# emilieparent/pypulsar

Hardware: AMD Instinct MI355X
Metric: DM-trial samples*channels/sec (node) + % HBM roofline (higher is better)
Workload: dtype u8

## Files before the change

### include/pdd.h

```cpp
#ifndef PDD_H
#define PDD_H

#include <stdint.h>

#ifdef __cplusplus
extern "C" {
#endif

enum { PDD_F32 = 0, PDD_U8 = 1, PDD_U16 = 2 };
enum {
  PDD_PAD_VALUE = 0,
  PDD_PAD_ROTATE = 1
};
enum { PDD_STAT_MEAN = 0, PDD_STAT_MEDIAN = 1, PDD_STAT_STD = 2, PDD_STAT_MIN = 3, PDD_STAT_MAX = 4 };
enum { PDD_LAYOUT_TIME_MAJOR = 0,
       PDD_LAYOUT_CHAN_MAJOR = 1   };

int pdd_version(void);
const char* pdd_last_error(void);
const char* pdd_source_digest(void);
int pdd_scratch_release(void);
int pdd_sync(void* stream);

int pdd_corner_turn(const void* in, int in_dtype, int64_t nspec, int64_t nchan, int64_t ld_in,
// ... 48 lines not shown
#define PDD_SWEEP_FACTOR_FORCE 2
#define PDD_SWEEP_FACTOR_G2 4
#define PDD_SWEEP_FACTOR_G4 8
#define PDD_SWEEP_NO_SKEW 16
int pdd_sweep_plan_create_ex(const int32_t* host_table, int64_t D, int64_t C, int dtype, int flags,
                             pdd_sweep_plan** plan);
int pdd_sweep_plan_factor(const pdd_sweep_plan* plan, int64_t* n_patterns);
int pdd_sweep_plan_skew(const pdd_sweep_plan* plan, int64_t* extra_tiles);
int pdd_sweep_execute(const pdd_sweep_plan* plan, const void* x, int64_t N, int64_t ld,
                      int pad_mode, const float* padvals, float* out, int64_t ld_out,
                      int64_t n_out, void* stream);
int pdd_sweep_execute_ex(const pdd_sweep_plan* plan, const void* x, int64_t N, int64_t ld,
                         int64_t piece, int64_t x_off, int pad_mode, const float* padvals,
                         float* out, int64_t ld_out, int64_t n_out, float out_bias,
                         void* stream);
int64_t pdd_sweep_pattern_bytes(const pdd_sweep_plan* plan, int64_t n_out);
int pdd_sweep_execute_stage(const pdd_sweep_plan* plan, const void* x, int64_t N, int64_t ld,
                            int64_t piece, int64_t x_off, int pad_mode, const float* padvals,
                            float* out, int64_t ld_out, int64_t n_out, float out_bias,
                            void* patterns, int64_t pattern_bytes, int stage, void* stream);
int pdd_stream_create_cu_mask(const uint32_t* mask, int n_words, void** stream);
int pdd_stream_destroy(void* stream);
int pdd_sweep_plan_create_grouped(const int32_t* host_table, int64_t n_grp, int64_t D, int64_t C,
                                  int dtype, pdd_sweep_plan** plan);
int pdd_sweep_execute_grouped(const pdd_sweep_plan* plan, const void* x, int64_t N, int64_t ld,
                              int pad_mode, const float* padvals, float* out, int64_t ld_out,
                              int64_t n_out, int64_t row_g, int64_t row_d, void* stream);
int pdd_sweep_execute_ds(const pdd_sweep_plan* plan, const uint8_t* x8, int64_t n_raw, int64_t ld,
                         int64_t ds, int pad_mode, const float* padvals, float* out,
                         int64_t ld_out, int64_t n_out, int64_t row_g, int64_t row_d,
// ... 80 lines not shown
```

### pypulsar_amd/_lib.py

```python
import ctypes
import os

import torch

from . import _digest

_HERE = os.path.dirname(os.path.abspath(__file__))
LIB_PATH = os.path.join(_HERE, "libpdd.so")
_DEV_LIB = os.environ.get("PDD_DEV_LIB")
if _DEV_LIB:
    LIB_PATH = _DEV_LIB

F32, U8, U16 = 0, 1, 2
PAD_VALUE, PAD_ROTATE = 0, 1
STAT_MEAN, STAT_MEDIAN, STAT_STD, STAT_MIN, STAT_MAX = 0, 1, 2, 3, 4
LAYOUT_TIME_MAJOR, LAYOUT_CHAN_MAJOR = 0, 1
ENOCHAIN = -5
ZDM_NONE, ZDM_INT, ZDM_WRAP = 0, 1, 2
SWEEP_FACTOR = 1
SWEEP_FACTOR_FORCE = 2
SWEEP_FACTOR_G2 = 4
SWEEP_FACTOR_G4 = 8
SWEEP_NO_SKEW = 16

# ... 3 lines not shown
    "pdd_zero_dm", "pdd_sweep_plan_create", "pdd_sweep_execute", "pdd_sweep_plan_info",
    "pdd_sweep_plan_set_input_max",
    "pdd_sweep_plan_destroy", "pdd_global_stats", "pdd_scale_rows", "pdd_masked_fill",
    "pdd_smooth", "pdd_zdm_downsample", "pdd_sweep_set_timing", "pdd_sweep_kernel_ms",
    "pdd_sweep_plan_create_grouped", "pdd_sweep_execute_grouped", "pdd_sp_chunk_stats",
    "pdd_sp_search", "pdd_psrfits_subints", "pdd_downsample_u8", "pdd_sweep_timing_read",
    "pdd_sweep_execute_ex", "pdd_zdm_int_downsample", "pdd_downsample_u8_u16",
    "pdd_sweep_execute_ds", "pdd_subband_chain", "pdd_scratch_release",
    "pdd_sweep_plan_create_ex", "pdd_sweep_plan_factor", "pdd_sweep_plan_skew", "pdd_source_digest",
    "pdd_sweep_plan_set_poison", "pdd_sweep_plan_set_segment_bytes",
    "pdd_sweep_pattern_bytes", "pdd_sweep_execute_stage", "pdd_stream_create_cu_mask",
    "pdd_stream_destroy", "pdd_ps_prep", "pdd_ps_block_medians", "pdd_ps_normalise",
    "pdd_ps_harmsum", "pdd_ps_search", "pdd_fold_rows", "pdd_fold_search",
    "pdd_acc_correlate", "pdd_acc_search", "pdd_rfi_stats_prep", "pdd_rfi_stats_power",
    "pdd_rfi_apply", "pdd_ffa_plan_info", "pdd_ffa_downsample", "pdd_ffa_detrend", "pdd_ffa_pass",
    "pdd_ffa_search",
)


def source_digest():
    return _digest.source_digest()


class PddLibraryMissing(RuntimeError):
    pass


class PddError(RuntimeError):
    pass


# ... 12 lines not shown
    "pdd_convert_f32": ([_vp, _int, _i64, _i64, _i64, _vp, _i64, _vp], _int),
    "pdd_channel_stats": ([_vp, _i64, _i64, _i64, _int, _vp, _vp], _int),
    "pdd_shift_pad": ([_vp, _i64, _i64, _i64, _vp, _int, _vp, _vp, _i64, _i64, _vp], _int),
    "pdd_shift_group_sum": ([_vp, _i64, _i64, _i64, _vp, _int, _vp, _i64, _vp, _i64, _i64, _vp],
                            _int),
    "pdd_downsample": ([_vp, _i64, _i64, _i64, _i64, _vp, _i64, _vp], _int),
    "pdd_downsample_u8": ([_vp, _i64, _i64, _i64, _i64, _vp, _i64, _vp], _int),
    "pdd_downsample_u8_u16": ([_vp, _i64, _i64, _i64, _i64, _vp, _i64, _vp], _int),
    "pdd_zero_dm": ([_vp, _int, _i64, _i64, _i64, _int, _vp, _i64, _vp], _int),
    "pdd_sweep_plan_create": ([_vp, _i64, _i64, _int, ctypes.POINTER(_vp)], _int),
    "pdd_sweep_plan_create_ex": ([_vp, _i64, _i64, _int, _int, ctypes.POINTER(_vp)], _int),
    "pdd_sweep_plan_factor": ([_vp, _vp], _int),
    "pdd_sweep_plan_skew": ([_vp, _vp], _int),
    "pdd_sweep_execute": ([_vp, _vp, _i64, _i64, _int, _vp, _vp, _i64, _i64, _vp], _int),
    "pdd_sweep_execute_ex": ([_vp, _vp, _i64, _i64, _i64, _i64, _int, _vp, _vp, _i64, _i64,
                              ctypes.c_float, _vp], _int),
    "pdd_sweep_plan_info": ([_vp, _vp], _int),
    "pdd_sweep_pattern_bytes": ([_vp, _i64], _i64),
    "pdd_sweep_execute_stage": ([_vp, _vp, _i64, _i64, _i64, _i64, _int, _vp, _vp, _i64, _i64,
                                 ctypes.c_float, _vp, _i64, _int, _vp], _int),
    "pdd_stream_create_cu_mask": ([_vp, _int, ctypes.POINTER(_vp)], _int),
    "pdd_stream_destroy": ([_vp], _int),
    "pdd_sweep_plan_set_input_max": ([_vp, _int], _int),
    "pdd_sweep_plan_destroy": ([_vp], _int),
    "pdd_global_stats": ([_vp, _i64, _i64, _i64, _vp, _vp], _int),
    "pdd_scale_rows": ([_vp, _i64, _i64, _i64, _vp, _i64, _vp, _i64, _vp, _i64, _vp], _int),
    "pdd_masked_fill": ([_vp, _i64, _i64, _i64, _vp, _i64, _vp, _vp, _i64, _vp], _int),
    "pdd_smooth": ([_vp, _i64, _i64, _i64, _i64, _int, _vp, _vp, _i64, _vp], _int),
    "pdd_zdm_downsample": ([_vp, _int, _i64, _i64, _i64, _i64, _int, _vp, _i64, _vp], _int),
    "pdd_zdm_int_downsample": ([_vp, _int, _i64, _i64, _i64, _i64, _int, _int, _vp, _i64, _vp],
# ... 105 lines not shown
```

### pypulsar_amd/csrc/pdd_sweep.hip

```cpp
#include <algorithm>
#include <cstdio>
#include <cstdlib>
#include <cstring>
#include <type_traits>
#include <vector>

#include "pdd_internal.h"
#include "sweep_plan.h"

namespace pdd {

template <bool U8, int S>
struct ElemOf {
  static constexpr int bytes = U8 ? 2 * S : 4 * S;
  static_assert(bytes == 8 || bytes == 16, "LDS element must be 8 or 16 bytes");
  using type = typename std::conditional<bytes == 8, uint2, uint4>::type;
};

__device__ __forceinline__ uint32_t get_w(const uint2& v, int i) { return i == 0 ? v.x : v.y; }
__device__ __forceinline__ uint32_t get_w(const uint4& v, int i) {
  return i == 0 ? v.x : (i == 1 ? v.y : (i == 2 ? v.z : v.w));
}
__device__ __forceinline__ void set_w(uint2& v, int i, uint32_t x) {
  if (i == 0) v.x = x; else v.y = x;
// ... 354 lines not shown
        "global_load_lds_dwordx4 %1, off\n\t"
        "s_mov_b32 m0, %0"
        : "=&s"(keep)
        : "v"(p), "s"(la)
        : "memory");
  }
}


constexpr int kIlPer = 4;
struct InLayout {
  int64_t ld;
  int64_t piece;
  int psh;
  int64_t pstride;
  __device__ __forceinline__ int64_t at(int c, int64_t s) const {
    return piece ? (s >> psh) * pstride + (int64_t)c * piece + (s & (piece - 1))
                 : (int64_t)c * ld + s;
  }
};

template <typename InT>
struct SrcRows {
  const InT* x;
  InLayout lay;
  __device__ __forceinline__ SrcRows(const void* xv, const InLayout& l)
      : x(static_cast<const InT*>(xv)), lay(l) {}
  __device__ __forceinline__ InT at(int c, int64_t s) const { return x[lay.at(c, s)]; }
};
template <int F, bool VEC>
struct SrcCoadd {
// ... 173 lines not shown

struct FxBatch {
  int y, z, w, lo, hi;
};
__device__ __forceinline__ FxBatch fx_batch(const int4* __restrict__ pat, const int* __restrict__ rng,
                                            int pb, int p1) {
  const int pl = min(pb + (int)(threadIdx.x & 63), p1 - 1);
  const int4 q = pat[pl];
  return {q.y, q.z, q.w, rng[2 * pl], rng[2 * pl + 1]};
}

struct FxS1Args : IlArgs {
  const int4* pat;
  const int* gtab;
  int NG;
};

struct FxFromImage {
  using El = ElemU16;
  static constexpr int kBlock = kFxE;
  static constexpr bool kNontemporal = false;
  const uint4* R;
  int64_t nR;
  __device__ __forceinline__ explicit FxFromImage(const FxS1Args& a)
      : R(static_cast<const uint4*>(a.x)), nR(a.nR) {}
  __device__ __forceinline__ void load_row(uint4* L, int c, int64_t i0, int W) const {
    for (int e = threadIdx.x; e < W; e += 256) {
      const int64_t i = i0 + e;
      L[e] = (i >= 0 && i < nR) ? R[(int64_t)c * nR + i] : make_uint4(0u, 0u, 0u, 0u);
    }
  }
};
template <typename InT>
struct FxFromInput {
  static constexpr bool kF32 = std::is_same<InT, float>::value;
  using El = typename std::conditional<kF32, ElemF32, ElemU16>::type;
  using V = typename El::value_t;
  static constexpr int kBlock = kF32 ? kFxEf : kFxE;
  static constexpr bool kNontemporal = !kF32;
  const SrcRows<InT> src;
  const FxS1Args& a;
  __device__ __forceinline__ explicit FxFromInput(const FxS1Args& a_) : src(a_.x, a_.lay), a(a_) {}
  __device__ __forceinline__ void load_row(typename El::elem_t* L, int c, int64_t i0, int W) const {
    const V pv = pad_value<V>(a.pad_mode, a.padvals, c);
    const int64_t s_lo = a.base + i0, s_hi = s_lo + W - 1 + (El::S - 1) * a.Qs;
// ... 6 lines not shown
        L[e] = El::pack(v);
      }
      return;
    }
    for (int e = threadIdx.x; e < W; e += 256) {
      const int64_t i = i0 + e;
      V v[El::S];
#pragma unroll
      for (int m = 0; m < El::S; ++m) {
        const int64_t sm = a.base + i + m * a.Qs;
        v[m] = (i < 0 || i >= a.nR) ? (V)0 : padded_sample<V>(src, c, sm, a.N, a.pad_mode, pv);
      }
      L[e] = El::pack(v);
    }
  }
};

template <typename Src, int FXG>
__global__ __launch_bounds__(256) void k_fx_stage1(const FxS1Args a) {
  using El = typename Src::El;
  using E = typename El::elem_t;
  constexpr int kE = Src::kBlock;
  extern __shared__ __attribute__((aligned(16))) unsigned char fx_smem[];
  E* L = reinterpret_cast<E*>(fx_smem);
  const int* __restrict__ gtab = a.gtab;
  const int4* __restrict__ pat = a.pat;
  E* __restrict__ P = static_cast<E*>(a.R);
  const int64_t nR = a.nR;
  const int NG = a.NG;
  const int g = blockIdx.x;
  const int64_t j0 = (int64_t)blockIdx.y * kE;
  const int p0 = gtab[g], p1 = gtab[g + 1];
  const int lo = gtab[NG + 1 + 2 * g], hi = gtab[NG + 2 + 2 * g];
  const int W = kE + hi - lo;
  const Src src(a);
  for (int k = 0; k < FXG; ++k) src.load_row(L + k * W, g * FXG + k, j0 + lo, W);
  __syncthreads();
  const int* rng = gtab + 3 * NG + 1;
  for (int pb = p0; pb < p1; pb += 64) {
    const FxBatch B = fx_batch(pat, rng, pb, p1);
    for (int i = 0; i < min(64, p1 - pb); ++i) {
      const int p = pb + i;
      const int4 q = make_int4(0, __builtin_amdgcn_readlane(B.y, i), __builtin_amdgcn_readlane(B.z, i),
                               __builtin_amdgcn_readlane(B.w, i));
      const int64_t jlo = __builtin_amdgcn_readlane(B.lo, i), jhi = nR + __builtin_amdgcn_readlane(B.hi, i);
      if (j0 >= jhi || j0 + kE <= jlo) continue;
#pragma unroll
      for (int e = threadIdx.x; e < kE; e += 256) {
        const int64_t j = j0 + e;
        if (j >= nR) break;
        E s = El::add(L[e - lo], L[W + e - lo + q.y]);
        if constexpr (FXG > 2) {
          s = El::add(s, L[2 * W + e - lo + q.z]);
          s = El::add(s, L[3 * W + e - lo + q.w]);
        }
        E* dst = P + (int64_t)p * nR + j;
        if constexpr (Src::kNontemporal) {
          typedef unsigned int u32x4v __attribute__((ext_vector_type(4)));
          const u32x4v sv = {s.x, s.y, s.z, s.w};
          __builtin_nontemporal_store(sv, reinterpret_cast<u32x4v*>(dst));
        } else {
          *dst = s;
        }
      }
    }
  }
}

typedef void (*fx_s1_fn)(FxS1Args);
constexpr int kFxImage = -1;
struct FxS1Instance {
  int src, fx;
  fx_s1_fn fn;
  int block;
};
#define PDD_FX_S1(SRC_, ...) \
  {SRC_, 2, k_fx_stage1<__VA_ARGS__, 2>, __VA_ARGS__::kBlock}, {SRC_, 4, k_fx_stage1<__VA_ARGS__, 4>, __VA_ARGS__::kBlock}
static const FxS1Instance kFxS1Instances[] = {
    PDD_FX_S1(kFxImage, FxFromImage), PDD_FX_S1(PDD_U8, FxFromInput<uint8_t>),
    PDD_FX_S1(PDD_U16, FxFromInput<uint16_t>), PDD_FX_S1(PDD_F32, FxFromInput<float>)};
#undef PDD_FX_S1

__device__ __forceinline__ int stage_il_dma_win(uint32_t lds_dst, const float4* src, int ne,
                                                int lane) {
  const int nq = (ne + 63) >> 6;
  uint32_t keep;
#define PDD_DMA_RUN(TEXT)                                                                      \
  asm volatile("s_mov_b32 %0, m0\n\ts_mov_b32 m0, %2\n\ts_nop 0\n\t" TEXT "s_mov_b32 m0, %0" \
               : "=&s"(keep) : "v"(s), "s"(m) : "memory")
  for (int q = 0; q < nq; q += 4) {
    const float4* s = src + q * 64 + lane;
    const uint32_t m = __builtin_amdgcn_readfirstlane(lds_dst + q * 1024);
// ... 533 lines not shown

static int debug_flags() { return 0; }

}

struct pdd_sweep_plan : pdd::PlanDims {
  int* d_tab = nullptr;
  int* d_bmin = nullptr;
  int* d_bspan = nullptr;
  int* d_pat = nullptr;
  int* d_wt = nullptr;
  int* d_gtab = nullptr;
  int* d_sig = nullptr;
  int input_max = 0;
  int poison = 0;
  int64_t seg_bytes = 0;
  static constexpr int kEvPairs = 1024;
  hipEvent_t* ev = nullptr;
  int timing = 0;
  int timed = 0;
  int dropped = 0;
};

using namespace pdd;

static void il_lohi(const pdd_sweep_plan* p, int64_t& lo, int64_t& hi) {
  if (p->fx) {
    lo = p->fx_lo;
    hi = (int64_t)p->fx_hi + p->fx_tpad;
  } else {
// ... 82 lines not shown
    const int J = 16 / ds;
    if ((uintptr_t)r.x % 16 == 0 && r.lay.ld % 16 == 0 && b0 % J == 0 && g.Qs % J == 0) vec = 16;
    else if ((uintptr_t)r.x % ds == 0 && r.lay.ld % ds == 0) vec = 1;
  }
  for (const IlInstance& k : kIlInstances) {
    if (k.ds != ds || k.vec != vec || k.dtype != p->dtype || k.u16 != (p->v.S == 8)) continue;
    const IlArgs a{r.x, r.lay, r.N, b0, g.Qs, g.nR, r.pad_mode, r.padvals, r.R};
    hipLaunchKernelGGL(k.fn, dim3((unsigned)cdiv(g.nR, k.per_block), (unsigned)C), dim3(256), 0,
                       r.st, a);
    return hipGetLastError() == hipSuccess ? 0 : il_launch_failed();
  }
  set_error("pdd_sweep_execute: no pre-pass kernel (downsample %d, dtype %d)", ds, p->dtype);
  return -3;
}

static int il_build_patterns(const IlRun& r, const IlSeg& g, int64_t t_base) {
  const pdd_sweep_plan* p = r.p;
  if (p->poison &&
      hipMemsetAsync(r.P, 0xFF, (size_t)(p->n_pat * g.nR) * sizeof(uint4), r.st) != hipSuccess)
    return il_launch_failed();
  if (hipMemsetAsync(r.P + p->n_pat * g.nR, 0, (size_t)g.nR * sizeof(uint4), r.st) != hipSuccess)
    return il_launch_failed();
  if (!p->d_gtab) {
    hipLaunchKernelGGL(k_fx_patterns, dim3((unsigned)p->n_pat, (unsigned)cdiv(g.nR, 256 * kIlPer)),
                       dim3(256), 0, r.st, (const uint4*)r.R, g.nR, (const int4*)p->d_pat, p->fx, r.P);
    return hipGetLastError() == hipSuccess ? 0 : il_launch_failed();
  }
  for (const FxS1Instance& k : kFxS1Instances) {
    if (k.src != (r.fx_direct ? p->dtype : kFxImage) || k.fx != p->fx) continue;
    const int NG = (int)(p->C / p->fx);
    const FxS1Args a{{r.fx_direct ? r.x : r.R, r.lay, r.N, t_base + g.lo + r.x_off, g.Qs, g.nR,
                      r.pad_mode, r.padvals, r.P},
                     (const int4*)p->d_pat, p->d_gtab, NG};
    hipLaunchKernelGGL(k.fn, dim3((unsigned)NG, (unsigned)cdiv(g.nR, k.block)), dim3(256),
                       (size_t)(p->fx * (k.block + p->fx_rspan)) * sizeof(uint4), r.st, a);
    return hipGetLastError() == hipSuccess ? 0 : il_launch_failed();
  }
  set_error("pdd_sweep_execute: no stage-1 kernel (groups of %d, dtype %d)", p->fx, p->dtype);
  return -3;
}

static int il_launch_sweep(const IlRun& r, const IlSeg& g, int64_t t_base, int64_t cnt, float* out,
                           int64_t ld_out, int64_t row_g, int64_t row_d, float out_bias, int flush_n) {
  const pdd_sweep_plan* p = r.p;
  const IlExtra& ex = r.ex;
  const int64_t blocks = g.n_tblk * p->n_dblk * p->n_grp;
  if (blocks >= (1ll << 31)) {
    set_error("pdd_sweep_execute: grid too large");
    return -1;
  }
// ... 91 lines not shown
  if (status != 0) {
    set_error("%s", err.c_str());
    return status;
  }
  pdd_sweep_plan* p = new pdd_sweep_plan();
  static_cast<PlanDims&>(*p) = sp;
  const bool il = p->v.kind == 0;
  hipError_t e = upload(&p->d_tab, il ? sp.meta : sp.rel);
  if (e == hipSuccess) e = upload(&p->d_bmin, il ? sp.chunks : sp.bmin);
  if (e == hipSuccess) e = upload(&p->d_bspan, sp.bspan);
  if (e == hipSuccess && p->fx) e = upload(&p->d_pat, sp.fxt.pat);
  if (e == hipSuccess && p->fx) e = upload(&p->d_wt, sp.fxt.wt);
  if (e == hipSuccess && p->fx_sig_max > 0) e = upload(&p->d_sig, sp.fxt.sig);
  if (e == hipSuccess && !sp.fxt.gtab.empty()) {
    e = upload(&p->d_gtab, sp.fxt.gtab);
    for (const FxS1Instance& k : kFxS1Instances)
      if (e == hipSuccess)
        e = hipFuncSetAttribute((const void*)k.fn, hipFuncAttributeMaxDynamicSharedMemorySize,
                                (int)(4 * (kFxEf + kFxRspan) * sizeof(uint4)));
  }
  if (e != hipSuccess) {
    set_error("pdd_sweep_plan_create: %s", hipGetErrorString(e));
    pdd_sweep_plan_destroy(p);
    return -2;
  }
  if (p->lds_bytes > 64 * 1024) {
    const void* kf = il ? (const void*)il_kernel_for(p->v, p->fx != 0) : (const void*)kernel_for(p->v);
    e = hipFuncSetAttribute(kf, hipFuncAttributeMaxDynamicSharedMemorySize, p->lds_bytes);
    if (e != hipSuccess) {
      set_error("pdd_sweep_plan_create: hipFuncSetAttribute: %s", hipGetErrorString(e));
      pdd_sweep_plan_destroy(p);
      return -2;
    }
  }
// ... 7 lines not shown
  int pad_mode;
  const float* padvals;
};
static int check_execute(const ExecShape& a) {
  PDD_REQUIRE(a.N >= a.N_min && a.n_out >= 0 && a.n_out <= a.n_out_max && a.ld_out >= a.n_out &&
                  a.x_off >= 0 && a.row_g >= 0 && a.row_d >= 0,
              "%s: bad shape", a.fn);
  PDD_REQUIRE(a.piece > 0 || a.ld >= a.ld_min, "%s: row stride %lld < %lld", a.fn, (long long)a.ld,
              (long long)a.ld_min);
  PDD_REQUIRE(a.piece == 0 || (a.piece & (a.piece - 1)) == 0, "%s: piece must be 2^k", a.fn);
  PDD_REQUIRE(a.pad_mode == PDD_PAD_ROTATE || (a.pad_mode == PDD_PAD_VALUE && a.padvals),
              "%s: bad pad mode %d", a.fn, a.pad_mode);
  return 0;
}
static InLayout in_layout(int64_t ld, int64_t piece = 0, int64_t C = 0) {
  InLayout lay{ld, piece, 0, C * piece};
  while ((1ll << lay.psh) < piece) ++lay.psh;
  return lay;
}
constexpr int64_t kAnyColumns = INT64_MAX;

extern "C" {

int pdd_sweep_plan_create(const int32_t* host_table, int64_t D, int64_t C, int dtype,
                          pdd_sweep_plan** plan_out) {
  return plan_create(host_table, 1, D, C, dtype, PDD_SWEEP_FACTOR, plan_out);
}

int pdd_sweep_plan_create_ex(const int32_t* host_table, int64_t D, int64_t C, int dtype, int flags,
                             pdd_sweep_plan** plan_out) {
  return plan_create(host_table, 1, D, C, dtype, flags, plan_out);
// ... 51 lines not shown
              "pdd_sweep_execute: the generic (sparse-grid) kernel reads channel-major input "
              "at offset 0 without an output bias");
  const int64_t n_tblk = cdiv(n_out, p->v.TB());
  const int64_t blocks = n_tblk * p->n_dblk;
  PDD_REQUIRE(blocks < (1ll << 31), "pdd_sweep_execute: grid too large");
  sweep_fn fn = kernel_for(p->v);
  PDD_REQUIRE(fn != nullptr, "pdd_sweep_execute: no kernel");
  hipLaunchKernelGGL(fn, dim3((unsigned)blocks), dim3(p->v.threads()), p->lds_bytes,
                     as_stream(stream), x, ld, (int)p->C, N, p->d_tab, (int)p->Dpad, (int)p->D,
                     p->d_bmin, p->d_bspan, pad_mode, padvals, out, ld_out, n_out, debug_flags(),
                     p->stride, (int)n_tblk, (int)p->n_dblk);
  PDD_LAUNCHED();
  return 0;
}

int64_t pdd_sweep_pattern_bytes(const pdd_sweep_plan* p, int64_t n_out) {
  PDD_REQUIRE(p && n_out >= 0, "pdd_sweep_pattern_bytes: bad arguments");
  if (!p->fx || !p->d_gtab || p->v.kind != 0) return 0;
  return (int64_t)(p->n_pat + 1) * il_seg(p, std::max<int64_t>(n_out, 1)).nR * 16;
}

int pdd_sweep_execute_stage(const pdd_sweep_plan* p, const void* x, int64_t N, int64_t ld,
                            int64_t piece, int64_t x_off, int pad_mode, const float* padvals,
                            float* out, int64_t ld_out, int64_t n_out, float out_bias,
                            void* patterns, int64_t pattern_bytes, int stage, void* stream) {
  PDD_REQUIRE(p && x && patterns && (out || stage == 1), "pdd_sweep_execute_stage: null pointer");
  PDD_REQUIRE(p->fx && p->d_gtab && p->v.kind == 0 && p->n_grp == 1,
              "pdd_sweep_execute_stage: needs a factorised single-group plan");
  PDD_REQUIRE(stage >= 1 && stage <= 3, "pdd_sweep_execute_stage: stage %d not 1, 2 or 3", stage);
  if (int rc = check_execute({"pdd_sweep_execute_stage", N, 1, ld, N, piece, x_off, n_out,
// ... 196 lines not shown
```

### pypulsar_amd/sharding.py

```python
import numpy as np
import torch
import torch.distributed as dist


def dm_slices(D, world, work=None):
    w = np.ones(D) if work is None else np.asarray(work, dtype=np.float64)
    assert len(w) == D and world >= 1
    cum = np.concatenate([[0.0], np.cumsum(w)])
    bounds = [0]
    for r in range(1, world):
        bounds.append(int(np.searchsorted(cum, cum[-1] * r / world, side="left")))
    bounds.append(D)
    bounds = np.maximum.accumulate(bounds)
    return [(int(bounds[r]), int(bounds[r + 1])) for r in range(world)]


def trial_work(dms, downsamp=1):
    d = np.broadcast_to(np.asarray(downsamp, dtype=np.float64), (len(dms),))
    return 1.0 / d


def plan_trial_work(ddplan):
    dms = np.concatenate([np.asarray(s.DMs, dtype=np.float64) for s in ddplan.DDsteps])
    work = np.concatenate([trial_work(s.DMs, s.downsamp) for s in ddplan.DDsteps])
# ... 26 lines not shown
    _all_gather_into(out, part.contiguous(), group=group)
    return out


def _codes():
    from . import _lib
    return {torch.uint8: _lib.U8, torch.float32: _lib.F32}


def _corner_turn(src_tc, dst_cm):
    from ._lib import call, ptr, stream_ptr
    n, C = src_tc.shape
    code = _codes()[src_tc.dtype]
    call("pdd_corner_turn", ptr(src_tc), code, n, C, src_tc.stride(0), ptr(dst_cm), code,
         dst_cm.stride(0), stream_ptr())


class DMShardedSweep(object):

    def __init__(self, dms, freqs, dt, N, dtype=torch.uint8, n_batches=1, work=None,
                 gather=False, dst=0, group=None, device=None, to_cm=None, sweep_fn=None,
                 pieces=None, world=None, rank=None, x_buf=None, gather_fn=None, factor=True):
        from . import delays as _delays
        self.group = group
        self.rehearse = world is not None
        if self.rehearse:
            self.world, self.rank = int(world), int(rank)
            assert 0 <= self.rank < self.world, "rank outside the rehearsed world"
            assert not gather, "a rehearsal has no plane gather (one device)"
        else:
# ... 19 lines not shown
        assert tab.size == 0 or tab.min() >= 0, "DM-sharded sweep expects delays >= 0"
        self.max_bin = int(tab.max()) if tab.size else 0
        self.n_out = self.N - self.max_bin
        assert self.n_out > 0 and self.T > self.max_bin, \
            "each time batch must be longer than the largest delay"
        edges = [0]
        for k in range(self.nb):
            edges.append(min(self.n_out, (k + 1) * self.T - self.max_bin))
        edges[-1] = self.n_out
        self.col_edges = edges
        self.slices = dm_slices(self.D, self.world, work)
        self.lo, self.hi = self.slices[self.rank]
        self.rows = self.hi - self.lo
        self.gather = bool(gather)
        self.dst = dst
        xshape = (self.N // self.P, self.C, self.P) if self.pieces else (self.C, self.N)
        if x_buf is not None:
            assert tuple(x_buf.shape) == xshape and x_buf.dtype == dtype and x_buf.is_contiguous()
            self.x = x_buf
        else:
            self.x = torch.empty(xshape, dtype=dtype, device=self.device)
        self.gather_fn = gather_fn
        assert gather_fn is None or self.pieces, "gather_fn takes the pieces layout"
        self.direct = self.rehearse and gather_fn is None
        if self.pieces:
            self.cm = ([] if self.direct else
                       [torch.empty((self.C, self.P), dtype=dtype, device=self.device)
                        for _ in range(2)])
            self.xt = None
        else:
            self.xt = (torch.empty((self.N, self.C), dtype=dtype, device=self.device)
                       if self.world > 1 and not self.rehearse else None)
        cols = [edges[k + 1] - edges[k] for k in range(self.nb)]
        if self.gather and self.rank == self.dst:
            self.full = [torch.empty((self.D, c), dtype=torch.float32, device=self.device)
                         for c in cols]
            self.planes = [f[self.lo:self.hi] for f in self.full]
        else:
            self.full = None
            self.planes = [torch.empty((self.rows, c), dtype=torch.float32, device=self.device)
                           for c in cols]
        self.to_cm = to_cm if to_cm is not None else _corner_turn
        self.sw = None
        if sweep_fn is None:
            from .sweep import DMSweep
            code = "u8" if dtype == torch.uint8 else "f32"
            if self.rows:
                self.sw = DMSweep(self.dms[self.lo:self.hi], self.freqs, dt, dtype=code,
                                  factor=factor)

            def sweep_fn(x, N, piece, x_off, dms_slice, out, n_cols):
                if piece:
                    self.sw.sweep_pieces(x, N, piece, x_off, n_cols, out)
                else:
                    self.sw(x[:, x_off:x_off + n_cols + self.max_bin], out=out, n_out=n_cols)
        self.sweep_fn = sweep_fn

    def __call__(self, part):
        nb = self.nb
        assert tuple(part.shape) == (nb, self.P, self.C) and part.dtype == self.dtype
        sends = []
        pending = [None] * nb
        for k in range(nb):
            pending[k] = self.exchange_batch(part, k)
            if k > 0:
                if pending[k - 1] is not None:
                    pending[k - 1].wait()
                sends.extend(self.sweep_batch(k - 1))
        if pending[nb - 1] is not None:
            pending[nb - 1].wait()
        sends.extend(self.sweep_batch(nb - 1))
        for w in sends:
            w.wait()
        return self.full if (self.gather and self.rank == self.dst) else self.planes

    def exchange_batch(self, part, k):
        W, T, P = self.world, self.T, self.P
        if self.direct:
            r = self.rank
            if self.pieces:
                self.to_cm(part[k], self.x[k * W + r])
            else:
                self.to_cm(part[k], self.x[:, k * T + r * P:k * T + (r + 1) * P])
            return None
        if self.pieces:
            dst = self.x[k * W:(k + 1) * W]
            if W == 1:
                self.to_cm(part[k], dst[0])
                return None
            cm = self.cm[k % 2]
            self.to_cm(part[k], cm)
            if self.gather_fn is not None:
                return self.gather_fn(dst.view(W * self.C, P), cm, k)
            return _all_gather_into(dst.view(W * self.C, P), cm, group=self.group,
                                    async_op=True)
        if W == 1:
            self.to_cm(part[k], self.x[:, k * T:(k + 1) * T])
            return None
        return _all_gather_into(self.xt[k * T:(k + 1) * T], part[k], group=self.group,
                                async_op=True)

    def sweep_batch(self, k):
        W, T = self.world, self.T
        if not self.pieces and W > 1 and not self.rehearse:
            self.to_cm(self.xt[k * T:(k + 1) * T], self.x[:, k * T:(k + 1) * T])
        a, b = self.col_edges[k], self.col_edges[k + 1]
        if self.rows and b > a:
            self.sweep_fn(self.x, self.N, self.P if self.pieces else 0, a,
                          self.dms[self.lo:self.hi], self.planes[k], b - a)
        return self._gather_batch(k) if self.gather else []

    def prefill(self, block_tc):
        assert tuple(block_tc.shape) == (self.N, self.C) and block_tc.dtype == self.dtype
        if self.pieces:
            for b in range(self.N // self.P):
                self.to_cm(block_tc[b * self.P:(b + 1) * self.P], self.x[b])
        else:
            self.to_cm(block_tc, self.x)

    def _gather_batch(self, k):
        if self.world == 1:
# ... 3 lines not shown
        works = []
        for r, (lo, hi) in enumerate(self.slices):
            if r != self.dst and hi > lo:
                works.append(dist.irecv(self.full[k][lo:hi], r, group=self.group))
        return works

    def plane(self):
        src = self.full if (self.gather and self.rank == self.dst) else self.planes
        return torch.cat(list(src), dim=1)

    def close(self):
        if self.sw is not None:
            self.sw.close()
            self.sw = None
        self.sweep_fn = None
        self.x = self.full = self.planes = None


def timeshard_edges(n_out, world, align=1024):
    edges = [0]
    for r in range(1, world):
        e = int(round(n_out * r / world / align)) * align
        edges.append(min(max(e, edges[-1]), n_out))
    edges.append(int(n_out))
    return edges


class TimeShardedSweep(object):

    def __init__(self, dms, freqs, dt, N, dtype=torch.uint8, world=None, rank=None, gather=False,
                 dst=0, group=None, device=None, to_cm=None, sweep_fn=None, factor=True,
# ... 211 lines not shown
```

### pypulsar_amd/sweep.py

```python
import ctypes

import numpy as np
import torch

from . import _lib
from ._lib import call, ptr, stream_ptr
from . import delays as _delays


_U16_TYPES = tuple(t for t in (torch.int16, getattr(torch, "uint16", None)) if t is not None)
_CODE_OF = {"f32": _lib.F32, "u8": _lib.U8, "u16": _lib.U16}
_PLAN_CODE = dict([(torch.float32, _lib.F32), (torch.uint8, _lib.U8)]
                  + [(t, _lib.U16) for t in _U16_TYPES])
_ANY_INPUT = dict.fromkeys(_PLAN_CODE)
_PIECES_INPUT = {torch.uint8: "u8", torch.float32: None}


def _plan_info(plan):
    a = np.zeros(8, dtype=np.int64)
    _lib.check(_lib.lib().pdd_sweep_plan_info(plan, a.ctypes.data_as(ctypes.c_void_p)),
               "pdd_sweep_plan_info")
    keys = ("D", "C", "dms_per_block", "samples_per_block", "lds_bytes", "max_bin", "min_bin",
            "variant")
    return dict(zip(keys, (int(v) for v in a)))
# ... 186 lines not shown
        n_out = self.n_out(N, True) if n_out is None else int(n_out)
        self._check_input(x8, {torch.uint8: "u16"}, out, n_out)
        if out is None:
            out = torch.empty((self.D, max(n_out, 1)), dtype=torch.float32, device=x8.device)
        call("pdd_sweep_execute_ds", self._plan(_lib.U16), ptr(x8), x8.shape[1], x8.stride(0),
             int(ds), mode, ptr(pv), ptr(out), out.stride(0), n_out, 0, 1, stream_ptr(stream))
        return out

    def sweep_pieces(self, xp, N, piece, x_off, n_out, out, stream=None):
        code = self._check_input(xp, _PIECES_INPUT, out, n_out, N, piece)
        ld = 0 if piece else xp.stride(0)
        call("pdd_sweep_execute_ex", self._plan(code), ptr(xp), N, ld, piece, x_off, _lib.PAD_VALUE,
             ptr(self._zero_pads(xp.device, stream)), ptr(out), out.stride(0), n_out, 0.0,
             stream_ptr(stream))
        return out

    def pattern_bytes(self, n_out, code=_lib.U8):
        return int(_lib.lib().pdd_sweep_pattern_bytes(self._plan(code), int(n_out)))

    def sweep_pieces_stage(self, xp, N, piece, x_off, n_out, out, patterns, stage, stream=None):
        code = self._check_input(xp, _PIECES_INPUT, out, n_out, N, piece)
        assert patterns.is_cuda and patterns.is_contiguous()
        nbytes = patterns.numel() * patterns.element_size()
        ld = 0 if piece else xp.stride(0)
        call("pdd_sweep_execute_stage", self._plan(code), ptr(xp), N, ld, piece, x_off,
             _lib.PAD_VALUE, ptr(self._zero_pads(xp.device, stream)), ptr(out),
             out.stride(0) if out is not None else 0, n_out, 0.0, ptr(patterns), nbytes, int(stage),
             stream_ptr(stream))
        return out

# ... 283 lines not shown
```

Before: 173600 billion.

## Add time-major direct stage-1 path and persistent XCD-aware prefetching stage-1 kernel

Adds a sweep entry point that reads time-major (time x channel) u8 input directly, so the single-device sharded sweep no longer needs a corner turn into a channel-major buffer. It also adds a persistent stage-1 kernel that takes work items from per-XCD atomic queues with an XCD-aware group ordering, and prefetches the next item's input into registers (word-wide u8 loads) while the current item's patterns are written. These target the extra transpose traffic, the launch and tail cost of the grid-per-item stage 1, and load latency. In exchange it adds queue atomics, more register pressure, a strided per-sample gather in time-major mode, and considerably more code paths.

After: 176700 billion, median of 6. 1.8% higher.

```diff
diff --git a/include/pdd.h b/include/pdd.h
--- a/include/pdd.h
+++ b/include/pdd.h
@@ -86,6 +86,9 @@
                          int64_t piece, int64_t x_off, int pad_mode, const float* padvals,
                          float* out, int64_t ld_out, int64_t n_out, float out_bias,
                          void* stream);
+int pdd_sweep_execute_tm(const pdd_sweep_plan* plan, const void* x, int64_t N, int64_t ld_t,
+                         int64_t x_off, int pad_mode, const float* padvals, float* out,
+                         int64_t ld_out, int64_t n_out, float out_bias, void* stream);
 int64_t pdd_sweep_pattern_bytes(const pdd_sweep_plan* plan, int64_t n_out);
 int pdd_sweep_execute_stage(const pdd_sweep_plan* plan, const void* x, int64_t N, int64_t ld,
                             int64_t piece, int64_t x_off, int pad_mode, const float* padvals,
diff --git a/pypulsar_amd/_lib.py b/pypulsar_amd/_lib.py
--- a/pypulsar_amd/_lib.py
+++ b/pypulsar_amd/_lib.py
@@ -41,7 +41,7 @@
     "pdd_ps_harmsum", "pdd_ps_search", "pdd_fold_rows", "pdd_fold_search",
     "pdd_acc_correlate", "pdd_acc_search", "pdd_rfi_stats_prep", "pdd_rfi_stats_power",
     "pdd_rfi_apply", "pdd_ffa_plan_info", "pdd_ffa_downsample", "pdd_ffa_detrend", "pdd_ffa_pass",
-    "pdd_ffa_search",
+    "pdd_ffa_search", "pdd_sweep_execute_tm",
 )
 
 
@@ -84,6 +84,8 @@
     "pdd_sweep_plan_skew": ([_vp, _vp], _int),
     "pdd_sweep_execute": ([_vp, _vp, _i64, _i64, _int, _vp, _vp, _i64, _i64, _vp], _int),
     "pdd_sweep_execute_ex": ([_vp, _vp, _i64, _i64, _i64, _i64, _int, _vp, _vp, _i64, _i64,
+                              ctypes.c_float, _vp], _int),
+    "pdd_sweep_execute_tm": ([_vp, _vp, _i64, _i64, _i64, _int, _vp, _vp, _i64, _i64,
                               ctypes.c_float, _vp], _int),
     "pdd_sweep_plan_info": ([_vp, _vp], _int),
     "pdd_sweep_pattern_bytes": ([_vp, _i64], _i64),
diff --git a/pypulsar_amd/csrc/fx_walk.h b/pypulsar_amd/csrc/fx_walk.h
--- /dev/null
+++ b/pypulsar_amd/csrc/fx_walk.h
@@ -0,0 +1,33 @@
+#pragma once
+#include <stdint.h>
+
+#if defined(__HIPCC__) || defined(__CUDACC__)
+#define PDD_FX_HD __host__ __device__
+#else
+#define PDD_FX_HD
+#endif
+
+namespace pdd {
+
+constexpr int kFxXcds = 8;
+constexpr int kFxWalkLine = 32;
+constexpr int kFxWalkRun = kFxXcds * kFxWalkLine;
+
+PDD_FX_HD inline int fx_walk_group(int s, int NG) {
+  const int full = NG / kFxWalkRun * kFxWalkRun;
+  if (s >= full) return s;
+  const int r = s % kFxWalkRun;
+  return s - r + (r % kFxXcds) * kFxWalkLine + r / kFxXcds;
+}
+
+struct FxWalkItem {
+  int group;
+  int64_t block;
+};
+PDD_FX_HD inline FxWalkItem fx_walk_item(int64_t i, int NG) {
+  return {fx_walk_group((int)(i % NG), NG), i / NG};
+}
+
+PDD_FX_HD inline int fx_walk_xcd(int64_t w) { return (int)(w % kFxXcds); }
+
+}
diff --git a/pypulsar_amd/csrc/pdd_sweep.hip b/pypulsar_amd/csrc/pdd_sweep.hip
--- a/pypulsar_amd/csrc/pdd_sweep.hip
+++ b/pypulsar_amd/csrc/pdd_sweep.hip
@@ -5,6 +5,7 @@
 #include <type_traits>
 #include <vector>
 
+#include "fx_walk.h"
 #include "pdd_internal.h"
 #include "sweep_plan.h"
 
@@ -392,7 +393,9 @@
   int64_t piece;
   int psh;
   int64_t pstride;
+  int64_t ld_t;
   __device__ __forceinline__ int64_t at(int c, int64_t s) const {
+    if (ld_t) return s * ld_t + c;
     return piece ? (s >> psh) * pstride + (int64_t)c * piece + (s & (piece - 1))
                  : (int64_t)c * ld + s;
   }
@@ -596,6 +599,10 @@
   const int4* pat;
   const int* gtab;
   int NG;
+  int64_t n_items;
+  unsigned int* queue;
+  int words;
+  int slot;
 };
 
 struct FxFromImage {
@@ -611,6 +618,12 @@
       const int64_t i = i0 + e;
       L[e] = (i >= 0 && i < nR) ? R[(int64_t)c * nR + i] : make_uint4(0u, 0u, 0u, 0u);
     }
+  }
+  __device__ __forceinline__ bool inner(int64_t i0, int W, int = 0) const {
+    return i0 >= 0 && i0 + W <= nR;
+  }
+  __device__ __forceinline__ uint4 elem(int c, int64_t i, bool in) const {
+    return (in || (i >= 0 && i < nR)) ? R[(int64_t)c * nR + i] : make_uint4(0u, 0u, 0u, 0u);
   }
 };
 template <typename InT>
@@ -647,31 +660,39 @@
       L[e] = El::pack(v);
     }
   }
+  __device__ __forceinline__ bool inner(int64_t i0, int W, int slack = 0) const {
+    const int64_t s_lo = a.base + i0, s_hi = s_lo + W - 1 + (El::S - 1) * a.Qs;
+    return i0 >= 0 && i0 + W <= a.nR && s_lo - slack >= 0 && s_hi + slack < a.N;
+  }
+  __device__ __forceinline__ typename El::elem_t elem(int c, int64_t i, bool in) const {
+    V v[El::S];
+    if (in) {
+#pragma unroll
+      for (int m = 0; m < El::S; ++m) v[m] = (V)src.at(c, a.base + i + m * a.Qs);
+    } else {
+      const V pv = pad_value<V>(a.pad_mode, a.padvals, c);
+#pragma unroll
+      for (int m = 0; m < El::S; ++m)
+        v[m] = (i < 0 || i >= a.nR) ? (V)0
+                                     : padded_sample<V>(src, c, a.base + i + m * a.Qs, a.N, a.pad_mode, pv);
+    }
+    return El::pack(v);
+  }
 };
 
 template <typename Src, int FXG>
-__global__ __launch_bounds__(256) void k_fx_stage1(const FxS1Args a) {
+__device__ __forceinline__ void fx_write_patterns(const FxS1Args& a, const typename Src::El::elem_t* L,
+                                                  int64_t j0, int p0, int p1, int lo, int W,
+                                                  const FxBatch& B0) {
   using El = typename Src::El;
   using E = typename El::elem_t;
   constexpr int kE = Src::kBlock;
-  extern __shared__ __attribute__((aligned(16))) unsigned char fx_smem[];
-  E* L = reinterpret_cast<E*>(fx_smem);
-  const int* __restrict__ gtab = a.gtab;
   const int4* __restrict__ pat = a.pat;
   E* __restrict__ P = static_cast<E*>(a.R);
   const int64_t nR = a.nR;
-  const int NG = a.NG;
-  const int g = blockIdx.x;
-  const int64_t j0 = (int64_t)blockIdx.y * kE;
-  const int p0 = gtab[g], p1 = gtab[g + 1];
-  const int lo = gtab[NG + 1 + 2 * g], hi = gtab[NG + 2 + 2 * g];
-  const int W = kE + hi - lo;
-  const Src src(a);
-  for (int k = 0; k < FXG; ++k) src.load_row(L + k * W, g * FXG + k, j0 + lo, W);
-  __syncthreads();
-  const int* rng = gtab + 3 * NG + 1;
+  const int* rng = a.gtab + 3 * a.NG + 1;
   for (int pb = p0; pb < p1; pb += 64) {
-    const FxBatch B = fx_batch(pat, rng, pb, p1);
+    const FxBatch B = pb == p0 ? B0 : fx_batch(pat, rng, pb, p1);
     for (int i = 0; i < min(64, p1 - pb); ++i) {
       const int p = pb + i;
       const int4 q = make_int4(0, __builtin_amdgcn_readlane(B.y, i), __builtin_amdgcn_readlane(B.z, i),
@@ -700,15 +721,237 @@
   }
 }
 
+template <typename Src, int FXG>
+__global__ __launch_bounds__(256) void k_fx_stage1(const FxS1Args a) {
+  using E = typename Src::El::elem_t;
+  constexpr int kE = Src::kBlock;
+  extern __shared__ __attribute__((aligned(16))) unsigned char fx_smem[];
+  E* L = reinterpret_cast<E*>(fx_smem);
+  const int* __restrict__ gtab = a.gtab;
+  const int NG = a.NG;
+  const int g = blockIdx.x;
+  const int64_t j0 = (int64_t)blockIdx.y * kE;
+  const int p0 = gtab[g], p1 = gtab[g + 1];
+  const int lo = gtab[NG + 1 + 2 * g], hi = gtab[NG + 2 + 2 * g];
+  const int W = kE + hi - lo;
+  const Src src(a);
+  for (int k = 0; k < FXG; ++k) src.load_row(L + k * W, g * FXG + k, j0 + lo, W);
+  __syncthreads();
+  if (p1 > p0)
+    fx_write_patterns<Src, FXG>(a, L, j0, p0, p1, lo, W,
+                                fx_batch(a.pat, gtab + 3 * NG + 1, p0, p1));
+}
+
+template <typename Src, int FXG>
+struct FxPreElems {
+  using E = typename Src::El::elem_t;
+  static constexpr int kWmax = Src::kBlock + 256;
+  static constexpr int kPer = (kWmax + 255) / 256;
+  E r[FXG][kPer];
+  __device__ __forceinline__ void fetch(const Src& src, int c0, int64_t i0, int W) {
+    if (W > kWmax) return;
+    const bool in = src.inner(i0, W);
+#pragma unroll
+    for (int k = 0; k < FXG; ++k)
+#pragma unroll
+      for (int n = 0; n < kPer; ++n) {
+        const int e = threadIdx.x + n * 256;
+        if (e < W) r[k][n] = src.elem(c0 + k, i0 + e, in);
+      }
+  }
+  __device__ __forceinline__ void commit(const Src& src, E* L, int c0, int64_t i0, int W) const {
+    if (W > kWmax) {
+      for (int k = 0; k < FXG; ++k) src.load_row(L + k * W, c0 + k, i0, W);
+      return;
+    }
+#pragma unroll
+    for (int k = 0; k < FXG; ++k)
+#pragma unroll
+      for (int n = 0; n < kPer; ++n) {
+        const int e = threadIdx.x + n * 256;
+        if (e < W) L[k * W + e] = r[k][n];
+      }
+  }
+};
+template <int FXG>
+struct FxPreWords {
+  using Src = FxFromInput<uint8_t>;
+  static constexpr int kWmax = kFxE + 256;
+  static constexpr int kUnits = FXG * ((kWmax + 3) / 4 + 1) > kWmax ? FXG * ((kWmax + 3) / 4 + 1) : kWmax;
+  static constexpr int kU = (kUnits + 255) / 256;
+  uint32_t d[kU][8];
+  int mode, sh, nq;
+  __device__ __forceinline__ void fetch(const Src& src, int c0, int64_t i0, int W) {
+    const FxS1Args& a = src.a;
+    const uint8_t* __restrict__ x = src.src.x;
+    const int64_t s0 = a.base + i0;
+    mode = 0;
+    if (!a.words || W > kWmax) return;
+    if (a.lay.ld_t) {
+      if (!src.inner(i0, W)) return;
+      mode = 2;
+#pragma unroll
+      for (int n = 0; n < kU; ++n) {
+        const int e = threadIdx.x + n * 256;
+        if (e < W) {
+#pragma unroll
+          for (int m = 0; m < 8; ++m) {
+            const uint8_t* q = x + (s0 + e + m * a.Qs) * a.lay.ld_t + c0;
+            if constexpr (FXG == 4) d[n][m] = *reinterpret_cast<const uint32_t*>(q);
+            else d[n][m] = *reinterpret_cast<const uint16_t*>(q);
+          }
+        }
+        __builtin_amdgcn_sched_barrier(0);
+      }
+      return;
+    }
+    if (!src.inner(i0, W, 3)) return;
+    mode = 1;
+    sh = (int)(s0 & 3);
+    nq = (W + sh + 3) >> 2;
+    if (a.lay.piece) fetch_rows<true>(a, x, c0, s0 - sh);
+    else fetch_rows<false>(a, x, c0, s0 - sh);
+  }
+  template <bool PIECES>
+  __device__ __forceinline__ void fetch_rows(const FxS1Args& a, const uint8_t* __restrict__ x, int c0,
+                                             int64_t sa) {
+#pragma unroll
+    for (int n = 0; n < kU; ++n) {
+      const int f = threadIdx.x + n * 256;
+      if (f < FXG * nq) {
+        const int k = f / nq, q = f - k * nq;
+        const int64_t s = sa + 4 * q;
+#pragma unroll
+        for (int m = 0; m < 8; ++m) {
+          const int64_t sm = s + m * a.Qs;
+          const int64_t o = PIECES ? (sm >> a.lay.psh) * a.lay.pstride + (int64_t)(c0 + k) * a.lay.piece +
+                                         (sm & (a.lay.piece - 1))
+                                   : (int64_t)(c0 + k) * a.lay.ld + sm;
+          d[n][m] = *reinterpret_cast<const uint32_t*>(x + o);
+        }
+      }
+      __builtin_amdgcn_sched_barrier(0);
+    }
+  }
+  __device__ __forceinline__ void commit(const Src& src, uint4* L, int c0, int64_t i0, int W) const {
+    if (mode == 0) {
+      for (int k = 0; k < FXG; ++k) src.load_row(L + k * W, c0 + k, i0, W);
+      return;
+    }
+    if (mode == 2) {
+#pragma unroll
+      for (int n = 0; n < kU; ++n) {
+        const int e = threadIdx.x + n * 256;
+        if (e < W) {
+#pragma unroll
+          for (int k = 0; k < FXG; ++k) {
+            uint32_t v[8];
+#pragma unroll
+            for (int m = 0; m < 8; ++m) v[m] = (d[n][m] >> (8 * k)) & 0xffu;
+            L[k * W + e] = ElemU16::pack(v);
+          }
+        }
+      }
+      return;
+    }
+#pragma unroll
+    for (int n = 0; n < kU; ++n) {
+      const int f = threadIdx.x + n * 256;
+      if (f < FXG * nq) {
+        const int k = f / nq, q = f - k * nq;
+#pragma unroll
+        for (int j = 0; j < 4; ++j) {
+          const int e = 4 * q - sh + j;
+          uint32_t v[8];
+#pragma unroll
+          for (int m = 0; m < 8; ++m) v[m] = (d[n][m] >> (8 * j)) & 0xffu;
+          if (e >= 0 && e < W) L[k * W + e] = ElemU16::pack(v);
+        }
+      }
+    }
+  }
+};
+
+struct FxItem {
+  int g, p0, p1, lo, W;
+  int64_t j0;
+};
+template <int kE>
+__device__ __forceinline__ FxItem fx_item(const FxS1Args& a, int i) {
+  const FxWalkItem w = fx_walk_item(i, a.NG);
+  const int* __restrict__ gtab = a.gtab;
+  const int g = w.group;
+  const int lo = gtab[a.NG + 1 + 2 * g], hi = gtab[a.NG + 2 + 2 * g];
+  return {g, gtab[g], gtab[g + 1], lo, kE + hi - lo, w.block * kE};
+}
+__device__ __forceinline__ int fx_take(unsigned int* queue, int xcd, unsigned int ticket, int n_items) {
+  for (int t = 0;; ++t) {
+    const int64_t i = (int64_t)ticket * kFxXcds + xcd;
+    if (i < n_items) return (int)i;
+    if (t == kFxXcds - 1) return -1;
+    xcd = (xcd + 1) % kFxXcds;
+    ticket = atomicAdd(queue + xcd, 1u);
+  }
+}
+
+template <typename Src, int FXG>
+__global__ __launch_bounds__(256, Src::kBlock == kFxE ? 4 : 2) void k_fx_stage1_p(const FxS1Args a) {
+  using E = typename Src::El::elem_t;
+  using Pre = typename std::conditional<std::is_same<Src, FxFromInput<uint8_t>>::value, FxPreWords<FXG>,
+                                        FxPreElems<Src, FXG>>::type;
+  constexpr int kE = Src::kBlock;
+  extern __shared__ __attribute__((aligned(16))) unsigned char fx_smem[];
+  E* L = reinterpret_cast<E*>(fx_smem);
+  int* slot = reinterpret_cast<int*>(fx_smem + a.slot);
+  const int n_items = (int)a.n_items;
+  const int xcd = fx_walk_xcd(blockIdx.x);
+  if (threadIdx.x == 0) {
+    slot[0] = fx_take(a.queue, xcd, atomicAdd(a.queue + xcd, 1u), n_items);
+    slot[1] = fx_take(a.queue, xcd, atomicAdd(a.queue + xcd, 1u), n_items);
+  }
+  __syncthreads();
+  const int first = __builtin_amdgcn_readfirstlane(slot[0]);
+  int nx = __builtin_amdgcn_readfirstlane(slot[1]);
+  if (first < 0) return;
+  const Src src(a);
+  Pre pre;
+  const int* rng = a.gtab + 3 * a.NG + 1;
+  FxItem cur = fx_item<kE>(a, first);
+  FxBatch Bc = {0, 0, 0, 0, 0};
+  if (cur.p1 > cur.p0) Bc = fx_batch(a.pat, rng, cur.p0, cur.p1);
+  pre.fetch(src, cur.g * FXG, cur.j0 + cur.lo, cur.W);
+  pre.commit(src, L, cur.g * FXG, cur.j0 + cur.lo, cur.W);
+  for (;;) {
+    __syncthreads();
+    FxItem nxt = cur;
+    FxBatch Bn = Bc;
+    if (nx >= 0) {
+      nxt = fx_item<kE>(a, nx);
+      if (nxt.p1 > nxt.p0) Bn = fx_batch(a.pat, rng, nxt.p0, nxt.p1);
+      pre.fetch(src, nxt.g * FXG, nxt.j0 + nxt.lo, nxt.W);
+    }
+    fx_write_patterns<Src, FXG>(a, L, cur.j0, cur.p0, cur.p1, cur.lo, cur.W, Bc);
+    if (nx < 0) break;
+    if (threadIdx.x == 0) slot[0] = fx_take(a.queue, xcd, atomicAdd(a.queue + xcd, 1u), n_items);
+    __syncthreads();
+    const int nn = __builtin_amdgcn_readfirstlane(slot[0]);
+    pre.commit(src, L, nxt.g * FXG, nxt.j0 + nxt.lo, nxt.W);
+    cur = nxt;
+    Bc = Bn;
+    nx = nn;
+  }
+}
+
 typedef void (*fx_s1_fn)(FxS1Args);
 constexpr int kFxImage = -1;
 struct FxS1Instance {
   int src, fx;
-  fx_s1_fn fn;
+  fx_s1_fn fn, fn_p;
   int block;
 };
-#define PDD_FX_S1(SRC_, ...) \
-  {SRC_, 2, k_fx_stage1<__VA_ARGS__, 2>, __VA_ARGS__::kBlock}, {SRC_, 4, k_fx_stage1<__VA_ARGS__, 4>, __VA_ARGS__::kBlock}
+#define PDD_FX_S1(SRC_, ...)                                                              \
+  {SRC_, 2, k_fx_stage1<__VA_ARGS__, 2>, k_fx_stage1_p<__VA_ARGS__, 2>, __VA_ARGS__::kBlock}, \
+  {SRC_, 4, k_fx_stage1<__VA_ARGS__, 4>, k_fx_stage1_p<__VA_ARGS__, 4>, __VA_ARGS__::kBlock}
 static const FxS1Instance kFxS1Instances[] = {
     PDD_FX_S1(kFxImage, FxFromImage), PDD_FX_S1(PDD_U8, FxFromInput<uint8_t>),
     PDD_FX_S1(PDD_U16, FxFromInput<uint16_t>), PDD_FX_S1(PDD_F32, FxFromInput<float>)};
@@ -1272,6 +1515,7 @@
   int* d_sig = nullptr;
   int input_max = 0;
   int poison = 0;
+  int fx_s1_wgs[2] = {0, 0};
   int64_t seg_bytes = 0;
   static constexpr int kEvPairs = 1024;
   hipEvent_t* ev = nullptr;
@@ -1384,6 +1628,16 @@
   return -3;
 }
 
+constexpr size_t kFxSlotBytes = 16;
+static size_t fx_s1_lds(const pdd_sweep_plan* p, const FxS1Instance& k) {
+  return (size_t)(p->fx * (k.block + p->fx_rspan)) * sizeof(uint4);
+}
+static bool fx_s1_words(const void* x, const InLayout& lay, int fx, int64_t Qs) {
+  const uintptr_t xa = (uintptr_t)x;
+  if (lay.ld_t) return xa % fx == 0 && lay.ld_t % fx == 0;
+  return xa % 4 == 0 && Qs % 4 == 0 && (lay.piece ? lay.piece % 4 == 0 : lay.ld % 4 == 0);
+}
+
 static int il_build_patterns(const IlRun& r, const IlSeg& g, int64_t t_base) {
   const pdd_sweep_plan* p = r.p;
   if (p->poison &&
@@ -1399,11 +1653,26 @@
   for (const FxS1Instance& k : kFxS1Instances) {
     if (k.src != (r.fx_direct ? p->dtype : kFxImage) || k.fx != p->fx) continue;
     const int NG = (int)(p->C / p->fx);
-    const FxS1Args a{{r.fx_direct ? r.x : r.R, r.lay, r.N, t_base + g.lo + r.x_off, g.Qs, g.nR,
-                      r.pad_mode, r.padvals, r.P},
-                     (const int4*)p->d_pat, p->d_gtab, NG};
-    hipLaunchKernelGGL(k.fn, dim3((unsigned)NG, (unsigned)cdiv(g.nR, k.block)), dim3(256),
-                       (size_t)(p->fx * (k.block + p->fx_rspan)) * sizeof(uint4), r.st, a);
+    FxS1Args a{{r.fx_direct ? r.x : r.R, r.lay, r.N, t_base + g.lo + r.x_off, g.Qs, g.nR,
+                r.pad_mode, r.padvals, r.P},
+               (const int4*)p->d_pat, p->d_gtab, NG, 0, nullptr, 0, 0};
+    const int64_t nblk = cdiv(g.nR, k.block);
+    const size_t lds = fx_s1_lds(p, k);
+    const int wgs = p->fx_s1_wgs[r.fx_direct];
+    a.n_items = NG * nblk;
+#ifndef PDD_FX_S1_ONESHOT
+    if (wgs > 0 && a.n_items > wgs && a.n_items < (1ll << 31) - 16ll * wgs) {
+      a.queue = static_cast<unsigned int*>(scratch(r.st, kScratchSmall, kFxXcds * sizeof(unsigned int)));
+      if (!a.queue) return -2;
+      if (hipMemsetAsync(a.queue, 0, kFxXcds * sizeof(unsigned int), r.st) != hipSuccess)
+        return il_launch_failed();
+      a.words = r.fx_direct && p->dtype == PDD_U8 && fx_s1_words(r.x, r.lay, p->fx, g.Qs);
+      a.slot = (int)lds;
+      hipLaunchKernelGGL(k.fn_p, dim3((unsigned)wgs), dim3(256), lds + kFxSlotBytes, r.st, a);
+      return hipGetLastError() == hipSuccess ? 0 : il_launch_failed();
+    }
+#endif
+    hipLaunchKernelGGL(k.fn, dim3((unsigned)NG, (unsigned)nblk), dim3(256), lds, r.st, a);
     return hipGetLastError() == hipSuccess ? 0 : il_launch_failed();
   }
   set_error("pdd_sweep_execute: no stage-1 kernel (groups of %d, dtype %d)", p->fx, p->dtype);
@@ -1525,10 +1794,23 @@
   if (e == hipSuccess && p->fx_sig_max > 0) e = upload(&p->d_sig, sp.fxt.sig);
   if (e == hipSuccess && !sp.fxt.gtab.empty()) {
     e = upload(&p->d_gtab, sp.fxt.gtab);
-    for (const FxS1Instance& k : kFxS1Instances)
+    int dev = 0, cus = 0;
+    if (e == hipSuccess) e = hipGetDevice(&dev);
+    if (e == hipSuccess) e = hipDeviceGetAttribute(&cus, hipDeviceAttributeMultiprocessorCount, dev);
+    for (const FxS1Instance& k : kFxS1Instances) {
+      const int lds_max = (int)(4 * (kFxEf + kFxRspan) * sizeof(uint4));
       if (e == hipSuccess)
-        e = hipFuncSetAttribute((const void*)k.fn, hipFuncAttributeMaxDynamicSharedMemorySize,
-                                (int)(4 * (kFxEf + kFxRspan) * sizeof(uint4)));
+        e = hipFuncSetAttribute((const void*)k.fn, hipFuncAttributeMaxDynamicSharedMemorySize, lds_max);
+      if (e == hipSuccess)
+        e = hipFuncSetAttribute((const void*)k.fn_p, hipFuncAttributeMaxDynamicSharedMemorySize,
+                                lds_max + (int)kFxSlotBytes);
+      if (e == hipSuccess && k.fx == p->fx && (k.src == kFxImage || k.src == p->dtype)) {
+        int per_cu = 0;
+        e = hipOccupancyMaxActiveBlocksPerMultiprocessor(&per_cu, (const void*)k.fn_p, 256,
+                                                         fx_s1_lds(p, k) + kFxSlotBytes);
+        p->fx_s1_wgs[k.src != kFxImage] = per_cu * cus;
+      }
+    }
   }
   if (e != hipSuccess) {
     set_error("pdd_sweep_plan_create: %s", hipGetErrorString(e));
@@ -1566,7 +1848,7 @@
   return 0;
 }
 static InLayout in_layout(int64_t ld, int64_t piece = 0, int64_t C = 0) {
-  InLayout lay{ld, piece, 0, C * piece};
+  InLayout lay{ld, piece, 0, C * piece, 0};
   while ((1ll << lay.psh) < piece) ++lay.psh;
   return lay;
 }
@@ -1648,6 +1930,22 @@
   return 0;
 }
 
+int pdd_sweep_execute_tm(const pdd_sweep_plan* p, const void* x, int64_t N, int64_t ld_t,
+                         int64_t x_off, int pad_mode, const float* padvals, float* out,
+                         int64_t ld_out, int64_t n_out, float out_bias, void* stream) {
+  PDD_REQUIRE(p && x && out, "pdd_sweep_execute_tm: null pointer");
+  if (int rc = check_execute({"pdd_sweep_execute_tm", N, 1, ld_t, p->C * p->n_grp, 0, x_off, n_out,
+                              kAnyColumns, ld_out, 0, 0, pad_mode, padvals}))
+    return rc;
+  if (n_out == 0) return 0;
+  PDD_REQUIRE(p->v.kind == 0, "pdd_sweep_execute_tm: the generic (sparse-grid) kernel reads "
+              "channel-major input");
+  InLayout lay = in_layout(0);
+  lay.ld_t = ld_t;
+  return execute_il(p, x, N, lay, x_off, pad_mode, padvals, out, ld_out, n_out, 0, 1, out_bias,
+                    stream);
+}
+
 int64_t pdd_sweep_pattern_bytes(const pdd_sweep_plan* p, int64_t n_out) {
   PDD_REQUIRE(p && n_out >= 0, "pdd_sweep_pattern_bytes: bad arguments");
   if (!p->fx || !p->d_gtab || p->v.kind != 0) return 0;
diff --git a/pypulsar_amd/sharding.py b/pypulsar_amd/sharding.py
--- a/pypulsar_amd/sharding.py
+++ b/pypulsar_amd/sharding.py
@@ -64,6 +64,9 @@
     code = _codes()[src_tc.dtype]
     call("pdd_corner_turn", ptr(src_tc), code, n, C, src_tc.stride(0), ptr(dst_cm), code,
          dst_cm.stride(0), stream_ptr())
+
+
+TIME_MAJOR_STAGE1 = True
 
 
 class DMShardedSweep(object):
@@ -113,8 +116,20 @@
         self.rows = self.hi - self.lo
         self.gather = bool(gather)
         self.dst = dst
+        self.sw = None
+        if sweep_fn is None and self.rows:
+            from .sweep import DMSweep
+            self.sw = DMSweep(self.dms[self.lo:self.hi], self.freqs, dt,
+                              dtype="u8" if dtype == torch.uint8 else "f32", factor=factor)
+        self.tm = bool(TIME_MAJOR_STAGE1 and self.world == 1 and not self.rehearse
+                       and self.sw is not None and to_cm is None and gather_fn is None
+                       and x_buf is None
+                       and self.sw.direct_stage1(_codes()[dtype]))
+        self._part = None
         xshape = (self.N // self.P, self.C, self.P) if self.pieces else (self.C, self.N)
-        if x_buf is not None:
+        if self.tm:
+            self.x = None
+        elif x_buf is not None:
             assert tuple(x_buf.shape) == xshape and x_buf.dtype == dtype and x_buf.is_contiguous()
             self.x = x_buf
         else:
@@ -123,7 +138,7 @@
         assert gather_fn is None or self.pieces, "gather_fn takes the pieces layout"
         self.direct = self.rehearse and gather_fn is None
         if self.pieces:
-            self.cm = ([] if self.direct else
+            self.cm = ([] if self.direct or self.tm else
                        [torch.empty((self.C, self.P), dtype=dtype, device=self.device)
                         for _ in range(2)])
             self.xt = None
@@ -140,14 +155,7 @@
             self.planes = [torch.empty((self.rows, c), dtype=torch.float32, device=self.device)
                            for c in cols]
         self.to_cm = to_cm if to_cm is not None else _corner_turn
-        self.sw = None
         if sweep_fn is None:
-            from .sweep import DMSweep
-            code = "u8" if dtype == torch.uint8 else "f32"
-            if self.rows:
-                self.sw = DMSweep(self.dms[self.lo:self.hi], self.freqs, dt, dtype=code,
-                                  factor=factor)
-
             def sweep_fn(x, N, piece, x_off, dms_slice, out, n_cols):
                 if piece:
                     self.sw.sweep_pieces(x, N, piece, x_off, n_cols, out)
@@ -175,6 +183,9 @@
 
     def exchange_batch(self, part, k):
         W, T, P = self.world, self.T, self.P
+        if self.tm:
+            self._part = part
+            return None
         if self.direct:
             r = self.rank
             if self.pieces:
@@ -204,6 +215,11 @@
         if not self.pieces and W > 1 and not self.rehearse:
             self.to_cm(self.xt[k * T:(k + 1) * T], self.x[:, k * T:(k + 1) * T])
         a, b = self.col_edges[k], self.col_edges[k + 1]
+        if self.tm:
+            if b > a:
+                self.sw.sweep_timemajor(self._part.reshape(self.N, self.C), self.N, a, b - a,
+                                        self.planes[k])
+            return []
         if self.rows and b > a:
             self.sweep_fn(self.x, self.N, self.P if self.pieces else 0, a,
                           self.dms[self.lo:self.hi], self.planes[k], b - a)
@@ -237,7 +253,7 @@
             self.sw.close()
             self.sw = None
         self.sweep_fn = None
-        self.x = self.full = self.planes = None
+        self.x = self.full = self.planes = self._part = None
 
 
 def timeshard_edges(n_out, world, align=1024):
diff --git a/pypulsar_amd/sweep.py b/pypulsar_amd/sweep.py
--- a/pypulsar_amd/sweep.py
+++ b/pypulsar_amd/sweep.py
@@ -224,6 +224,22 @@
              ptr(self._zero_pads(xp.device, stream)), ptr(out), out.stride(0), n_out, 0.0,
              stream_ptr(stream))
         return out
+
+    def sweep_timemajor(self, x_tc, N, x_off, n_out, out, stream=None):
+        if x_tc.dim() != 2 or x_tc.shape[1] != self.C or x_tc.stride(1) != 1 or x_tc.shape[0] < N:
+            raise ValueError("expected a [>= %d, C=%d] device tensor with unit channel stride"
+                             % (N, self.C))
+        if x_tc.dtype not in _PLAN_CODE:
+            raise TypeError("%s input: a sweep takes float32, uint8 or 16-bit samples" % x_tc.dtype)
+        if out.shape[0] != self.D or out.shape[1] < n_out or out.stride(1) != 1:
+            raise ValueError("out must be [D=%d, >= %d] with unit column stride" % (self.D, n_out))
+        call("pdd_sweep_execute_tm", self._plan(_PLAN_CODE[x_tc.dtype]), ptr(x_tc), N,
+             x_tc.stride(0), x_off, _lib.PAD_VALUE, ptr(self._zero_pads(x_tc.device, stream)),
+             ptr(out), out.stride(0), n_out, 0.0, stream_ptr(stream))
+        return out
+
+    def direct_stage1(self, code=_lib.U8):
+        return self.pattern_bytes(1, code) > 0
 
     def pattern_bytes(self, n_out, code=_lib.U8):
         return int(_lib.lib().pdd_sweep_pattern_bytes(self._plan(code), int(n_out)))
```
